# wagnva/semantic-nerf-for-satellite-data

Hardware: AMD Instinct MI355X
Metric: train rays/sec (4096 rays x 64 samples) (higher is better)
Workload: dtype f32(f16x2)

## Files before the change

### semantic-nerf-for-satellite-data_amd/csrc/api.hip

```cpp
#include <stdarg.h>
#include <stdio.h>
#include <stdlib.h>
#include <string.h>

#include <mutex>

#include "aux_kernels.h"
#include "bsp.h"
#include "composite.h"
#include "gemm.h"
#include "plan.h"

namespace snerf {

int forward_bsp(const Plan& p, const float* pk, const SnerfInputs* in, const SnerfOutputs* out, void* workspace, hipStream_t st);
int backward_bsp(const Plan& p, const float* pk, const SnerfInputs* in, const SnerfOutGrads* go, float* gp, float* d_t, float* d_t_s,
                 void* workspace, hipStream_t st);

static thread_local char g_err[512] = "";
void set_error(const char* fmt, ...) {
  va_list ap;
  va_start(ap, fmt);
  vsnprintf(g_err, sizeof(g_err), fmt, ap);
  va_end(ap);
// ... 269 lines not shown
namespace {
struct BufNote { const void* p; bool composed; };
constexpr int NOTE_MAX = 256;
BufNote g_notes[NOTE_MAX];
int g_n_notes = 0, g_note_next = 0;
std::mutex g_note_mu;
void note_plan(const void* buf, bool composed) {
  std::lock_guard<std::mutex> lk(g_note_mu);
  for (int i = 0; i < g_n_notes; ++i) if (g_notes[i].p == buf) { g_notes[i].composed = composed; return; }
  if (g_n_notes < NOTE_MAX) g_notes[g_n_notes++] = {buf, composed};
  else { g_notes[g_note_next] = {buf, composed}; g_note_next = (g_note_next + 1) % NOTE_MAX; }
}
int check_plan_note(const void* buf, bool composed, const char* who, const char* what) {
  std::lock_guard<std::mutex> lk(g_note_mu);
  for (int i = 0; i < g_n_notes; ++i)
    if (g_notes[i].p == buf && g_notes[i].composed != composed) {
      set_error("%s: the %s was written under SNERF_COMPOSE_FEATS=%d, this call is planned with %d (pack, forward and backward must agree)",
                who, what, g_notes[i].composed ? 1 : 0, composed ? 1 : 0);
      return SNERF_ERR_BAD_DESC;
    }
  return SNERF_OK;
}
}

static int check_inputs(const Plan& p, const SnerfInputs* in) {
  if (!in) { set_error("null inputs"); return SNERF_ERR_NULL; }
  if (!in->sun_d || in->sun_stride < 3) { set_error("sun_d (N,3) with stride >= 3 is required"); return SNERF_ERR_NULL; }
  if (!in->t) { set_error("t (N,tau) is required"); return SNERF_ERR_NULL; }
  if (p.x_ts >= 0 && !in->t_s) { set_error("t_s is required with use_separate_tj_for_semantic"); return SNERF_ERR_NULL; }
  if (in->xyz) {
    if (!in->z_vals) { set_error("explicit xyz needs explicit z_vals"); return SNERF_ERR_NULL; }
  } else {
    if (!in->rays) { set_error("rays or xyz is required"); return SNERF_ERR_NULL; }
    if (!in->z_vals && !in->z_steps) { set_error("z_steps is required when z_vals is not given"); return SNERF_ERR_NULL; }
  }
  return SNERF_OK;
}

}

using namespace snerf;

extern "C" {

int snerf_version(void) { return SNERF_ABI_VERSION; }
const char* snerf_last_error(void) { return g_err; }

size_t snerf_packed_floats(const SnerfDesc* desc) {
  Plan p;
  if (make_plan(desc, &p)) return 0;
  return p.packed_floats;
}

size_t snerf_grad_floats(const SnerfDesc* desc) {
  Plan p;
  if (make_plan(desc, &p)) return 0;
  return p.n_fp32;
}

size_t snerf_workspace_bytes(const SnerfDesc* desc) {
  Plan p;
  if (make_plan(desc, &p)) return 0;
  return p.ws_bytes;
}

int snerf_pack_params(const SnerfDesc* desc, const SnerfParams* params, float* packed, void* stream) {
  Plan p;
  RC(make_plan(desc, &p));
  if (!params || !packed) { set_error("null params/packed"); return SNERF_ERR_NULL; }
  TableBuilder tb;
  build_tables(p, params, tb);
  if (tb.missing) { set_error("snerf_pack_params: a parameter tensor required by this SnerfDesc is NULL"); return SNERF_ERR_NULL; }
  hipStream_t st = (hipStream_t)stream;
  RC(launch_zero_bytes(packed, p.n_fp32 * sizeof(float), st));
  for (int i = 0; i < tb.nt; ++i) RC(launch_copy_table(tb.tabs[i], packed, 0, st));
  char* planes = reinterpret_cast<char*>(packed + p.n_fp32);
  int* exps = reinterpret_cast<int*>(planes + p.wp_bytes);
  unsigned* maxbits = reinterpret_cast<unsigned*>(exps + bsp::WPACK_MAX);
  note_plan(packed, p.compose_feats);
  if (!p.compose_feats) return bsp::launch_wpack(p.wj, packed, planes, exps, maxbits, p.pl, st);
  {
    bsp::SgTable tb;
    bsp::compose_jobs(tb, packed + p.w_h1, packed + p.w_fs, packed + p.b_fs, packed + p.b_h1, packed + p.o_wc, packed + p.o_bc, p.W, p.FA, p.N1);
    RC(bsp::launch_sgemm(tb, 64, st));
  }
  bsp::WPackTable first, rest;
  first.n = rest.n = 0;
  for (int i = 0; i < p.wj.n; ++i) (i < p.wj_first ? first.j[first.n++] : rest.j[rest.n++]) = p.wj.j[i];
  RC(bsp::launch_wpack(first, packed, planes, exps, maxbits, p.pl, st));
  return bsp::launch_wpack(rest, packed, planes, exps, maxbits, p.pl, st);
}

int snerf_unpack_grads(const SnerfDesc* desc, const float* packed_grads, const SnerfParams* grads, int accumulate,
                       void* stream) {
  Plan p;
  RC(make_plan(desc, &p));
  if (!grads || !packed_grads) { set_error("null grads"); return SNERF_ERR_NULL; }
  TableBuilder tb;
  build_tables(p, grads, tb);
  if (tb.missing) { set_error("snerf_unpack_grads: a gradient tensor required by this SnerfDesc is NULL"); return SNERF_ERR_NULL; }
  hipStream_t st = (hipStream_t)stream;
  for (int i = 0; i < tb.nt; ++i) RC(launch_copy_table(tb.tabs[i], const_cast<float*>(packed_grads), accumulate ? 2 : 1, st));
  return SNERF_OK;
}

int snerf_forward(const SnerfDesc* desc, const float* packed_params, const SnerfInputs* in, const SnerfOutputs* out,
                  void* workspace, size_t workspace_bytes, void* stream) {
  Plan p;
  RC(make_plan(desc, &p));
  if (!packed_params || !out || !workspace) { set_error("snerf_forward: null argument"); return SNERF_ERR_NULL; }
  if (workspace_bytes < p.ws_bytes) { set_error("snerf_forward: workspace too small (%zu < %zu)", workspace_bytes, p.ws_bytes); return SNERF_ERR_WORKSPACE; }
  if (((uintptr_t)workspace & 255) || ((uintptr_t)packed_params & 255)) { set_error("workspace and packed params must be 256-byte aligned"); return SNERF_ERR_WORKSPACE; }
  RC(check_inputs(p, in));
  RC(check_plan_note(packed_params, p.compose_feats, "snerf_forward", "packed parameter buffer"));
  note_plan(workspace, p.compose_feats);
  return forward_bsp(p, packed_params, in, out, workspace, (hipStream_t)stream);
}

int snerf_backward(const SnerfDesc* desc, const float* packed_params, const SnerfInputs* in, const SnerfOutGrads* gout,
                   float* packed_grads, float* d_t, float* d_t_s, void* workspace, size_t workspace_bytes, void* stream) {
  Plan p;
  RC(make_plan(desc, &p));
  if (!p.train) { set_error("snerf_backward needs the SnerfDesc used for the SNERF_FLAG_TRAIN forward"); return SNERF_ERR_BAD_DESC; }
  if (!packed_params || !gout || !packed_grads || !workspace) { set_error("snerf_backward: null argument"); return SNERF_ERR_NULL; }
  if (workspace_bytes < p.ws_bytes) { set_error("snerf_backward: workspace too small (%zu < %zu)", workspace_bytes, p.ws_bytes); return SNERF_ERR_WORKSPACE; }
  if (((uintptr_t)workspace & 255) || ((uintptr_t)packed_params & 255) || ((uintptr_t)packed_grads & 255)) { set_error("workspace and packed buffers must be 256-byte aligned"); return SNERF_ERR_WORKSPACE; }
  RC(check_inputs(p, in));
  RC(check_plan_note(packed_params, p.compose_feats, "snerf_backward", "packed parameter buffer"));
  RC(check_plan_note(workspace, p.compose_feats, "snerf_backward", "workspace"));
  return backward_bsp(p, packed_params, in, gout, packed_grads, d_t, d_t_s, workspace, (hipStream_t)stream);
}

int snerf_sample_z(const float* rays, const float* z_steps, const float* u, float* z, int n_rays, int n_samples, void* stream) {
  if (!rays || !z_steps || !z || n_rays <= 0 || n_samples <= 0) { set_error("snerf_sample_z: bad argument"); return SNERF_ERR_NULL; }
  return launch_sample_z(rays, z_steps, u, z, n_rays, n_samples, (hipStream_t)stream);
}

int snerf_embedding_rows(const float* table, int n_embed, int tau, const long long* idx, int n, float* rows, void* stream) {
  if (!table || !idx || !rows || n_embed <= 0 || tau <= 0 || n <= 0) { set_error("snerf_embedding_rows: bad argument"); return SNERF_ERR_NULL; }
  return launch_embedding_rows(table, n_embed, tau, idx, n, rows, (hipStream_t)stream);
}

int snerf_embedding_backward(const long long* idx, const float* d_rows, int n, int tau, int n_embed, float* grad_table, void* stream) {
  if (!idx || !d_rows || !grad_table || n_embed <= 0 || tau <= 0 || n <= 0) { set_error("snerf_embedding_backward: bad argument"); return SNERF_ERR_NULL; }
  return launch_embedding_backward(idx, d_rows, n, tau, n_embed, grad_table, (hipStream_t)stream);
}

int snerf_profile_begin(void) { return profile_begin(); }
int snerf_profile_end(SnerfProfile* out) { return profile_end(out); }

}
```

### semantic-nerf-for-satellite-data_amd/csrc/bsp.h

```cpp
#pragma once
#include "common.h"
#include "gemm.h"

namespace snerf {
namespace bsp {

constexpr int RB = 128;
constexpr int CB = 128;
constexpr int E_MAX = 100;
constexpr int E_QUIET = 60;

typedef __amdgpu_buffer_rsrc_t srd_t;
typedef unsigned int u32x4 __attribute__((ext_vector_type(4)));
typedef unsigned int u32x2 __attribute__((ext_vector_type(2)));
typedef _Float16 f16x8 __attribute__((ext_vector_type(8)));
typedef _Float16 f16x4 __attribute__((ext_vector_type(4)));
constexpr unsigned OOB = 0xFFFFFFF0u;

__host__ __device__ inline int ncb_of(int ld) { return (ld + CB - 1) / CB; }
__host__ __device__ inline size_t plane_bytes(size_t rows, int ld, int pl = 2) { return rows * (size_t)ld * 2 * pl; }
__host__ __device__ inline size_t etab_ints(size_t rows, int ld) { return ((rows + RB - 1) / RB) * (size_t)ncb_of(ld); }
__host__ __device__ inline unsigned g16_off(int k, int pl = 2) { return (unsigned)(k >> 4) * 32u * (unsigned)pl + (unsigned)(k & 15) * 2u; }

__host__ __device__ inline int exp_of_maxbits(unsigned b) {
// ... 77 lines not shown
  float* colsum = nullptr; int ldcs = 0;
  int tiles_i = 0, tiles_j = 0;
  int tj_skip = -1;
  int tiles_jr = 0;
  int rev = 0;
  int dbg = 0;
  int* tile_ctr = nullptr;
  int pl = 2;
  const float* nd_w = nullptr; float* nd_out = nullptr; unsigned long long nd_stride = 0;
  int nd_omax = 0, nd_ldw = 0;
  int nd_rows[8] = {0, 0, 0, 0, 0, 0, 0, 0}, nd_row0[8] = {0, 0, 0, 0, 0, 0, 0, 0}, nd_woff[8] = {0, 0, 0, 0, 0, 0, 0, 0};
};
__host__ __device__ inline size_t sign_words(size_t rows, int ld) { return ((rows + 31) / 32) * (size_t)((ld + 63) / 64) * 64; }

struct DwArgs {
  const char* A = nullptr; const int* EA = nullptr; int lda = 0; int a_col0 = 0;
  const char* B = nullptr; const int* EB = nullptr; int ldb = 0; int b_col0 = 0;
  int I = 0, J = 0, P = 0;
  float* C = nullptr; int ldc = 0;
  int k_split = 0, n_split = 1; unsigned long long slab_stride = 0;
  int tiles_i = 0, tiles_j = 0;
  int pl = 2;
};

constexpr int TR_MAXL = 8;
constexpr int TR_SLOTS = TR_MAXL + 1;
struct TrunkArgs {
  const char* pe = nullptr; const int* Epe = nullptr;
  int P = 0, W = 0, L = 0; unsigned skip_mask = 0;
  int gamma_free_layer = 0;
  const char* Wp[TR_SLOTS] = {}; const int* EW[TR_SLOTS] = {}; unsigned w_bytes[TR_SLOTS] = {}; int K[TR_SLOTS] = {};
  const float* bias[TR_SLOTS] = {}; float w0[TR_SLOTS] = {};
  char* F = nullptr; int* EF = nullptr; int ldf = 0;
  char* H[TR_MAXL] = {}; int* EH[TR_MAXL] = {}; unsigned* Hsign[TR_MAXL] = {};
  const float* nd_w = nullptr; float* nd_out = nullptr; unsigned long long nd_stride = 0;
  int* tile_ctr = nullptr;
  int dbg = 0;
};
inline int trunk_gamma_free_layer(int L, unsigned skip_mask) {
  int g = 2;
  for (int l = 2; l < L; ++l)
    if ((skip_mask >> l) & 1u) g = l;
  return g < L - 1 ? g : L - 1;
}
inline bool trunk_dma_in_final_layer(int L, unsigned skip_mask, bool feats_fused) {
  return !feats_fused && trunk_gamma_free_layer(L, skip_mask) == L - 1;
}
int launch_trunk(const TrunkArgs& a, bool train, hipStream_t st);
void trunk_set_grid_override(int n);
void trunk_set_fusion(int on);
bool trunk_fusion_enabled();

int launch_kc(const KcArgs& a, hipStream_t st);
void kc_set_grid_override(int n);
int launch_kc_narrow(const KcArgs& a, hipStream_t st);
int launch_dw(const DwArgs& a, bool narrow_i, hipStream_t st);

int launch_to_planes(const float* src, int ld_src, int rows, int cols, char* dst, int* E, int ld, int col0, int pl, hipStream_t st);
int launch_from_planes(const char* src, const int* E, int ld, int col0, int rows, int cols, float* dst, int ld_dst, int pl, hipStream_t st);

struct WPackJob {
  unsigned long long src_off;
  int src_ld;
  int rows, K;
  int transposed;
  unsigned long long dst_off;
  int e_idx;
  int m_rows, m_cols;
};
constexpr int WPACK_MAX = 48;
struct WPackTable { WPackJob j[WPACK_MAX]; int n; };
constexpr int WPACK_CHUNK = 24;
struct WPackChunk { WPackJob j[WPACK_CHUNK]; int n; };
__host__ __device__ inline size_t wp16_bytes(int rows, int K, int pl = 2) { return (size_t)((rows + 31) / 32) * (size_t)(K / 16) * 1024 * pl; }
int launch_wpack(const WPackTable& tb, const float* master, char* planes, int* exps, unsigned* maxbits, int pl, hipStream_t st);

struct SgJob {
  const float* A = nullptr; long long sa_i = 0, sa_k = 0;
  const float* B = nullptr; long long sb_k = 0, sb_j = 0;
  const float* D = nullptr; int ldd = 0;
  const float* u = nullptr; const float* v = nullptr;
  float* C = nullptr; int ldc = 0;
  int M = 0, N = 0, K = 0, acc = 0;
  int blk0 = 0;
};
constexpr int SG_MAX = 6;
struct SgTable { SgJob j[SG_MAX]; int n = 0; };
int launch_sgemm(const SgTable& tb, int tile_m, hipStream_t st);
void compose_jobs(SgTable& tb, const float* w_h1, const float* w_f, const float* b_f, const float* b_h1, float* wc, float* bc, int W, int FA, int N1);
void uncompose_jobs(SgTable& tb, const float* G, const float* gc, const float* w_h1, const float* w_f, const float* b_f,
                    float* dw_h1, float* db_h1, float* dw_f, float* db_f, int W, int FA, int M);

}
struct EncodeArgs;
namespace bsp {
int launch_encode_bsp(const EncodeArgs& a, char* pe, int* Epe, char* fa, int* Efa, int fa_col0, int pl, hipStream_t st);
int launch_zero_cols(char* base, size_t pitch, size_t width_bytes, int rows, hipStream_t st);
int launch_colsum32_bsp(const float* in, int rows, float* partial, char* planes, int* E, int pl, hipStream_t st);

}
}
```

### semantic-nerf-for-satellite-data_amd/csrc/bsp_aux.hip

```cpp
#include "bsp.h"
#include "aux_kernels.h"

namespace snerf {
namespace bsp {

__device__ __forceinline__ float block_max_256(float m, float* sm) {
#pragma unroll
  for (int o = 32; o >= 1; o >>= 1) m = fmaxf(m, __shfl_xor(m, o, 64));
  __syncthreads();
  if ((threadIdx.x & 63) == 0) sm[threadIdx.x >> 6] = m;
  __syncthreads();
  return fmaxf(fmaxf(sm[0], sm[1]), fmaxf(sm[2], sm[3]));
}

__global__ __launch_bounds__(256) void to_planes_kernel(const float* __restrict__ src, int ld_src, int rows, int cols,
                                                        char* __restrict__ dst, int* __restrict__ E, int ld, int col0, int pl) {
  __shared__ float sm[4];
  const int rb = blockIdx.y, cb = blockIdx.x;
  const int t = threadIdx.x, c8 = cb * 128 + (t & 15) * 8;
  float v[8][8];
  float m = 0.f;
#pragma unroll
  for (int i = 0; i < 8; ++i) {
    const int r = rb * 128 + (t >> 4) + 16 * i;
// ... 26 lines not shown
    set_error("to_planes: bad argument (ld % 16, col0 % 128)");
    return SNERF_ERR_BAD_DESC;
  }
  hipLaunchKernelGGL(to_planes_kernel, dim3((cols + 127) / 128, (rows + 127) / 128), dim3(256), 0, st, src, ld_src, rows, cols,
                     dst, E, ld, col0, pl);
  SNERF_LAUNCH_CHECK();
  return SNERF_OK;
}

__global__ void from_planes_kernel(const char* __restrict__ src, const int* __restrict__ E, int ld, int col0, int rows, int cols,
                                   float* __restrict__ dst, int ld_dst, int pl) {
  const size_t g = (size_t)blockIdx.x * blockDim.x + threadIdx.x;
  if (g >= (size_t)rows * cols) return;
  const int r = (int)(g / cols), c = (int)(g - (size_t)r * cols);
  const char* p = src + (size_t)r * ld * 2 * pl + g16_off(col0 + c, pl);
  const float hi = (float)*reinterpret_cast<const _Float16*>(p), lo = pl == 2 ? (float)*reinterpret_cast<const _Float16*>(p + 32) : 0.f;
  const int e = E[(size_t)(r >> 7) * ncb_of(ld) + ((col0 + c) >> 7)];
  dst[(size_t)r * ld_dst + c] = __builtin_amdgcn_ldexpf(hi + lo, -e);
}

int launch_from_planes(const char* src, const int* E, int ld, int col0, int rows, int cols, float* dst, int ld_dst, int pl, hipStream_t st) {
  const size_t n = (size_t)rows * cols;
  hipLaunchKernelGGL(from_planes_kernel, dim3((unsigned)((n + 255) / 256)), dim3(256), 0, st, src, E, ld, col0, rows, cols, dst, ld_dst, pl);
  SNERF_LAUNCH_CHECK();
  return SNERF_OK;
}

__global__ __launch_bounds__(256) void wmax_kernel(WPackChunk tb, const float* __restrict__ master, unsigned* __restrict__ maxbits) {
  const WPackJob j = tb.j[blockIdx.y];
  if (j.transposed == 1) return;
  float m = 0.f;
  const int wave = threadIdx.x >> 6, lane = threadIdx.x & 63;
  for (int r = blockIdx.x * 4 + wave; r < j.m_rows; r += gridDim.x * 4) {
    const float* row = master + j.src_off + (size_t)r * j.src_ld;
    for (int c = lane; c < j.m_cols; c += 64) m = fmaxf(m, fabsf(row[c]));
  }
#pragma unroll
  for (int o = 32; o >= 1; o >>= 1) m = fmaxf(m, __shfl_xor(m, o, 64));
  if ((threadIdx.x & 63) == 0 && m > 0.f) atomicMax(maxbits + j.e_idx, __float_as_uint(m));
}

__global__ __launch_bounds__(256) void wpack_kernel(WPackChunk tb, const float* __restrict__ master, char* __restrict__ planes,
                                                    int* __restrict__ exps, const unsigned* __restrict__ maxbits, int pl) {
  const WPackJob j = tb.j[blockIdx.y];
  const int rb32 = (j.rows + 31) >> 5, nks = j.K >> 4;
  const int e = exp_of_maxbits(maxbits[j.e_idx]);
  if (blockIdx.x == 0 && threadIdx.x == 0) exps[j.e_idx] = e;
  const float sc = pow2f(e);
  for (int unit = blockIdx.x; unit < rb32 * nks; unit += gridDim.x) {
    const int ks = unit / rb32, ub = unit - ks * rb32;
    const int r = threadIdx.x >> 3, kp = (threadIdx.x & 7) * 2;
    const int ra = ub * 32 + wf16_row(r), ka = ks * 16 + kp;
    float x[2];
#pragma unroll
    for (int q = 0; q < 2; ++q) {
      const int k = ka + q;
      const bool ok = j.transposed ? (k < j.m_rows && ra < j.m_cols) : (ra < j.m_rows && k < j.m_cols);
      x[q] = ok ? master[j.src_off + (j.transposed ? (size_t)k * j.src_ld + ra : (size_t)ra * j.src_ld + k)] : 0.f;
    }
    const _Float16 h0 = (_Float16)(x[0] * sc), h1 = (_Float16)(x[1] * sc);
    const _Float16 l0 = (_Float16)(x[0] * sc - (float)h0), l1 = (_Float16)(x[1] * sc - (float)h1);
    typedef _Float16 f16x2 __attribute__((ext_vector_type(2)));
    char* u = planes + j.dst_off + (size_t)unit * 1024 * pl + (32 * (kp >> 3) + r) * 16 + (kp & 7) * 2;
    *reinterpret_cast<f16x2*>(u) = f16x2{h0, h1};
    if (pl == 2) *reinterpret_cast<f16x2*>(u + 1024) = f16x2{l0, l1};
  }
}

int launch_wpack(const WPackTable& tb, const float* master, char* planes, int* exps, unsigned* maxbits, int pl, hipStream_t st) {
  if (tb.n <= 0) return SNERF_OK;
  { int rc = launch_zero_bytes(maxbits, WPACK_MAX * sizeof(unsigned), st); if (rc) return rc; }
  for (int pass = 0; pass < 2; ++pass)
    for (int first = 0; first < tb.n; first += WPACK_CHUNK) {
      WPackChunk c;
      c.n = tb.n - first < WPACK_CHUNK ? tb.n - first : WPACK_CHUNK;
      for (int i = 0; i < c.n; ++i) c.j[i] = tb.j[first + i];
      if (pass == 0) hipLaunchKernelGGL(wmax_kernel, dim3(32, c.n), dim3(256), 0, st, c, master, maxbits);
      else hipLaunchKernelGGL(wpack_kernel, dim3(128, c.n), dim3(256), 0, st, c, master, planes, exps, maxbits, pl);
      SNERF_LAUNCH_CHECK();
    }
  return SNERF_OK;
}

template <int TM>
__global__ __launch_bounds__(256) void sgemm_jobs_kernel(const SgTable tb) {
  constexpr int BM = 16 * TM, BN = 64, BK = 16;
  __shared__ float As[BK][BM + 1];
  __shared__ float Bs[BK][BN + 4];
  int q = 0;
  while (q + 1 < tb.n && (int)blockIdx.x >= tb.j[q + 1].blk0) ++q;
  const SgJob jb = tb.j[q];
  const int tiles_n = (jb.N + BN - 1) / BN;
  const int tile = (int)blockIdx.x - jb.blk0;
  const int i0 = (tile / tiles_n) * BM, j0 = (tile % tiles_n) * BN;
  const int t = threadIdx.x, ty = t >> 4, tx = t & 15;
  float acc[TM][4];
#pragma unroll
  for (int r = 0; r < TM; ++r)
#pragma unroll
    for (int c = 0; c < 4; ++c) acc[r][c] = 0.f;
  const bool a_k_fast = jb.sa_k == 1, b_j_fast = jb.sb_j == 1;
  for (int k0 = 0; k0 < jb.K; k0 += BK) {
#pragma unroll
    for (int s = 0; s < (BM * BK) / 256; ++s) {
      const int idx = t + 256 * s;
      const int i = a_k_fast ? idx / BK : idx % BM, k = a_k_fast ? idx % BK : idx / BM;
      As[k][i] = (i0 + i < jb.M && k0 + k < jb.K) ? jb.A[(long long)(i0 + i) * jb.sa_i + (long long)(k0 + k) * jb.sa_k] : 0.f;
    }
#pragma unroll
    for (int s = 0; s < (BN * BK) / 256; ++s) {
      const int idx = t + 256 * s;
      const int j = b_j_fast ? idx % BN : idx / BK, k = b_j_fast ? idx / BN : idx % BK;
      Bs[k][j] = (j0 + j < jb.N && k0 + k < jb.K) ? jb.B[(long long)(k0 + k) * jb.sb_k + (long long)(j0 + j) * jb.sb_j] : 0.f;
    }
    __syncthreads();
#pragma unroll
    for (int k = 0; k < BK; ++k) {
      float a[TM], b[4];
#pragma unroll
      for (int r = 0; r < TM; ++r) a[r] = As[k][ty * TM + r];
#pragma unroll
      for (int c = 0; c < 4; ++c) b[c] = Bs[k][tx * 4 + c];
#pragma unroll
      for (int r = 0; r < TM; ++r)
#pragma unroll
        for (int c = 0; c < 4; ++c) acc[r][c] = fmaf(a[r], b[c], acc[r][c]);
    }
    __syncthreads();
  }
#pragma unroll
  for (int r = 0; r < TM; ++r) {
    const int i = i0 + ty * TM + r;
    if (i >= jb.M) continue;
#pragma unroll
    for (int c = 0; c < 4; ++c) {
      const int j = j0 + tx * 4 + c;
      if (j >= jb.N) continue;
      float x = acc[r][c];
      if (jb.u) x = fmaf(jb.u[i], jb.v[j], x);
      if (jb.D) x += jb.D[(size_t)i * jb.ldd + j];
      float* o = jb.C + (size_t)i * jb.ldc + j;
      *o = jb.acc ? *o + x : x;
    }
  }
}

void compose_jobs(SgTable& tb, const float* w_h1, const float* w_f, const float* b_f, const float* b_h1, float* wc, float* bc, int W, int FA, int N1) {
  const int X = FA - W;
  tb.n = 0;
  auto job = [&]() -> SgJob& { tb.j[tb.n] = SgJob(); return tb.j[tb.n++]; };
  { SgJob& j = job(); j.A = w_h1; j.sa_i = FA; j.sa_k = 1; j.B = w_f; j.sb_k = W; j.sb_j = 1; j.C = wc; j.ldc = FA; j.M = N1; j.N = W; j.K = W; }
  { SgJob& j = job(); j.D = w_h1 + W; j.ldd = FA; j.C = wc + W; j.ldc = FA; j.M = N1; j.N = X; }
  { SgJob& j = job(); j.D = w_f + (size_t)W * W; j.ldd = W; j.C = wc + (size_t)N1 * FA; j.ldc = FA; j.M = 32; j.N = W; }
  { SgJob& j = job(); j.C = wc + (size_t)N1 * FA + W; j.ldc = FA; j.M = 32; j.N = X; }
  { SgJob& j = job(); j.A = w_h1; j.sa_i = FA; j.sa_k = 1; j.B = b_f; j.sb_k = 1; j.sb_j = 0; j.D = b_h1; j.ldd = 1; j.C = bc; j.ldc = 1; j.M = N1; j.N = 1; j.K = W; }
}
void uncompose_jobs(SgTable& tb, const float* G, const float* gc, const float* w_h1, const float* w_f, const float* b_f,
                    float* dw_h1, float* db_h1, float* dw_f, float* db_f, int W, int FA, int M) {
  tb.n = 0;
  auto job = [&]() -> SgJob& { tb.j[tb.n] = SgJob(); return tb.j[tb.n++]; };
  { SgJob& j = job(); j.A = G; j.sa_i = FA; j.sa_k = 1; j.B = w_f; j.sb_k = 1; j.sb_j = W; j.u = gc; j.v = b_f; j.C = dw_h1; j.ldc = FA; j.M = M; j.N = W; j.K = W; j.acc = 1; }
  { SgJob& j = job(); j.A = w_h1; j.sa_i = 1; j.sa_k = FA; j.B = G; j.sb_k = FA; j.sb_j = 1; j.C = dw_f; j.ldc = W; j.M = W; j.N = W; j.K = M; j.acc = 1; }
  { SgJob& j = job(); j.A = w_h1; j.sa_i = 1; j.sa_k = FA; j.B = gc; j.sb_k = 1; j.sb_j = 0; j.C = db_f; j.ldc = 1; j.M = W; j.N = 1; j.K = M; j.acc = 1; }
  { SgJob& j = job(); j.D = gc; j.ldd = 1; j.C = db_h1; j.ldc = 1; j.M = M; j.N = 1; j.acc = 1; }
}

int launch_sgemm(const SgTable& tb0, int tile_m, hipStream_t st) {
  if (tb0.n <= 0) return SNERF_OK;
  if (tb0.n > SG_MAX || (tile_m != 64 && tile_m != 32)) { set_error("sgemm: bad job table"); return SNERF_ERR_BAD_DESC; }
  SgTable tb = tb0;
  int blocks = 0;
  for (int q = 0; q < tb.n; ++q) {
    SgJob& j = tb.j[q];
    if (!j.C || j.M <= 0 || j.N <= 0 || j.K < 0 || j.ldc < 1 || (j.K > 0 && (!j.A || !j.B)) || (j.u && !j.v) || (j.D && j.ldd < 1)) {
      set_error("sgemm: bad job %d", q);
      return SNERF_ERR_BAD_DESC;
    }
    j.blk0 = blocks;
    blocks += ((j.M + tile_m - 1) / tile_m) * ((j.N + 63) / 64);
  }
  if (tile_m == 64) hipLaunchKernelGGL(sgemm_jobs_kernel<4>, dim3(blocks), dim3(256), 0, st, tb);
  else hipLaunchKernelGGL(sgemm_jobs_kernel<2>, dim3(blocks), dim3(256), 0, st, tb);
  SNERF_LAUNCH_CHECK();
  return SNERF_OK;
}

__global__ void zero_cols_kernel(char* base, size_t pitch, int width16, int rows) {
  const int i = blockIdx.x * blockDim.x + threadIdx.x;
  if (i >= rows * width16) return;
  const int r = i / width16, c = i - r * width16;
  *reinterpret_cast<u32x4*>(base + (size_t)r * pitch + 16 * (size_t)c) = u32x4{0u, 0u, 0u, 0u};
}
int launch_zero_cols(char* base, size_t pitch, size_t width_bytes, int rows, hipStream_t st) {
  const int w16 = (int)(width_bytes / 16);
  if (w16 <= 0 || rows <= 0) return SNERF_OK;
  hipLaunchKernelGGL(zero_cols_kernel, dim3((unsigned)(((size_t)rows * w16 + 255) / 256)), dim3(256), 0, st, base, pitch, w16, rows);
  SNERF_LAUNCH_CHECK();
  return SNERF_OK;
}

__device__ __forceinline__ void point_xyz(const EncodeArgs& a, long long point, float (&x)[3]) {
  const int n = (int)((unsigned)point / (unsigned)a.S);
#pragma unroll
  for (int c = 0; c < 3; ++c) {
    if (a.xyz != nullptr) {
      x[c] = a.xyz[point * 3 + c];
    } else {
#pragma clang fp contract(off)
      const float o = a.rays[n * 8 + c];
      const float d = a.dir_is_sun ? a.sun_d[(size_t)n * a.sun_stride + c] : a.rays[n * 8 + 3 + c];
      const float dz = d * a.z[point];
      x[c] = o + dz;
    }
  }
}
__device__ __forceinline__ float extras_value(const EncodeArgs& a, int n, int c) {
  if (c >= a.x_sun && c < a.x_sun + 3) return a.sun_d[(size_t)n * a.sun_stride + (c - a.x_sun)];
  if (a.t != nullptr && c >= a.x_t && c < a.x_t + a.tau) return a.t[(size_t)n * a.tau + (c - a.x_t)];
  if (a.t_s != nullptr && a.x_ts >= 0 && c >= a.x_ts && c < a.x_ts + a.tau) return a.t_s[(size_t)n * a.tau + (c - a.x_ts)];
  return 0.f;
}

struct EncodeBsp {
  EncodeArgs a;
  char* pe; int* Epe;
  char* fa; int* Efa; int fa_col0;
  int pl;
};

__global__ __launch_bounds__(256) void encode_bsp_kernel(EncodeBsp g) {
  __shared__ float sm[4];
  const EncodeArgs& a = g.a;
  const int rb = blockIdx.x, t = threadIdx.x;
  if (rb == 0) for (int i = t; i < a.zero_n; i += 256) a.zero[i] = 0u;
  const long long P = (long long)a.N * a.S;
  const long long p0 = (long long)rb * 128;
  const int npts = (int)min((long long)128, P - p0);
  float mx = 0.f, me = 0.f;
  if (a.F == 0)
    for (int i = t; i < npts; i += 256) {
      float x[3];
      point_xyz(a, p0 + i, x);
      mx = fmaxf(mx, fmaxf(fabsf(x[0]), fmaxf(fabsf(x[1]), fabsf(x[2]))));
    }
  if (g.fa != nullptr) {
    const int n0 = (int)((unsigned)p0 / (unsigned)a.S), n1 = (int)((unsigned)(p0 + npts - 1) / (unsigned)a.S);
    for (int i = t; i < (n1 - n0 + 1) * 16; i += 256) me = fmaxf(me, fabsf(extras_value(a, n0 + (i >> 4), i & 15)));
  }
  const int e_pe = a.F > 0 ? 13 : exp_of_maxbits(__float_as_uint(block_max_256(mx, sm)));
  const int e_x = g.fa != nullptr ? exp_of_maxbits(__float_as_uint(block_max_256(me, sm))) : 0;
  if (t == 0) {
    g.Epe[rb] = e_pe;
    if (g.fa != nullptr) g.Efa[(size_t)rb * ncb_of(a.FA) + (g.fa_col0 >> 7)] = e_x;
  }
  const float s_pe = pow2f(e_pe), s_x = pow2f(e_x);
  const int gpe = a.Ep >> 4, ngrp = gpe + (g.fa != nullptr ? 1 : 0);
  for (int item = t; item < npts * ngrp; item += 256) {
    const int pl = item / ngrp, grp = item - pl * ngrp;
    const long long point = p0 + pl;
    float v[16];
    char* d;
    float sc;
    if (grp < gpe) {
      float x[3];
      point_xyz(a, point, x);
// ... 118 lines not shown
```

### semantic-nerf-for-satellite-data_amd/csrc/bsp_pass.hip

```cpp
#include "aux_kernels.h"
#include "bsp.h"
#include "composite.h"
#include "plan.h"

namespace snerf {

namespace {
struct Ws {
  char* base;
  char* c(size_t off) const { return base + off; }
  float* f(size_t off) const { return reinterpret_cast<float*>(base + off); }
  int* i(size_t off) const { return reinterpret_cast<int*>(base + off); }
  unsigned* u(size_t off) const { return reinterpret_cast<unsigned*>(base + off); }
  void a(bsp::KcArgs& g, const PlaneT& t, int k, int col0 = 0) const { g.A = c(t.o); g.EA = i(t.e); g.lda = t.ld; g.a_col0 = col0; g.Ka = k; }
  void a2(bsp::KcArgs& g, const PlaneT& t) const { g.A2 = c(t.o); g.EA2 = i(t.e); g.lda2 = t.ld; }
  void out(bsp::KcArgs& g, const PlaneT& t, int col0 = 0) const { g.C = c(t.o); g.EC = i(t.e); g.ldc = t.ld; g.c_col0 = col0; g.Csign = t.s ? u(t.s) : nullptr; }
  void h(bsp::KcArgs& g, const PlaneT& t, int col0 = 0) const { g.H = c(t.o); g.EH = i(t.e); g.ldh = t.ld; g.h_col0 = col0; g.Hsign = t.s ? u(t.s) : nullptr; }
  void dz(bsp::DwArgs& g, const PlaneT& t) const { g.A = c(t.o); g.EA = i(t.e); g.lda = t.ld; g.a_col0 = 0; }
  void x(bsp::DwArgs& g, const PlaneT& t, int col0) const { g.B = c(t.o); g.EB = i(t.e); g.ldb = t.ld; g.b_col0 = col0; }
};
struct WOp { const char* W; const int* EW; int rb32; unsigned bytes; int K; };
WOp wop(const Plan& p, const float* pk, int job) {
  const char* planes = reinterpret_cast<const char*>(pk + p.n_fp32);
  const bsp::WPackJob& w = p.wj.j[job];
// ... 315 lines not shown
    const int r0 = p.sc ? p.sun_col : 0;
    const int nt = (P + 127) / 128, X = p.FA - W;
    RC(dw_gemm(r.w_h1, dz1, p.h1w, false, p.fa, 0, p.FA));
    RC(red_add_elem2d(rq.elem, r.w_h1.slab + W, r.w_h1.sp.ns, r.w_h1.stride, p.h1w, X, p.FA, gp + p.w_h1 + (size_t)r0 * p.FA + W, p.FA));
    RC(red_add_elem2d(rq.elem, r.w_h1.slab, r.w_h1.sp.ns, r.w_h1.stride, p.h1w, W, p.FA, r.w_h1.slab, p.FA));
    RC(red_store_last(rq.elem));
    RC(red_add_col(rq.col, r.cs_fin, nt, (size_t)r.ld_cs1, p.h1w, r.cs_fin));
    RC(red_store_last(rq.col));
    uncompose = true;
    RC(transient_grads());
    if (sig_live) {
      RC(narrow_grad(dsig, r.nar_sig, p.pdsig, gp + p.b_fs + W));
      RC(dw_gemm(r.w_fs, p.pdsig, NARROW, true, hl, 0, W));
      RC(dw_reduce(r.w_fs, (size_t)NARROW * W, gp + p.w_fs + (size_t)W * W));
    }
    { const PlaneT sw = dz_cur; dz_cur = dz_nxt; dz_nxt = sw; }
    bsp::KcArgs g;
    ws.a(g, dz1, p.h1w);
    if (sig_live) ws.a2(g, p.pdsig);
    weights(g, p, pk, p.wj_th1, 0, r0); g.I = P; g.J = W; g.K = sig_live ? p.h1w + NARROW : p.h1w;
    ws.out(g, dz_cur);
    dact(g, hl, 0, (p.L == 1) ? 30.f : 1.f);
    colsum(g, r.cs_hl, W);
    RC(launch_kc(g));
    RC(bias_from_colsum(r.cs_hl, W, gp + p.b_tr[p.L - 1]));
  }
  const PlaneT dfa = p.dzb.view(p.FA);
  if (!p.compose_feats) {
    const int r0 = p.sc ? p.sun_col : 0;
    RC(dw_gemm(r.w_h1, dz1, p.h1w, false, p.fa, 0, p.FA));
    RC(dw_reduce(r.w_h1, (size_t)p.h1w * p.FA, gp + p.w_h1 + (size_t)r0 * p.FA));
    bsp::KcArgs g;
    ws.a(g, dz1, p.h1w); weights(g, p, pk, p.wj_th1, 0, r0);
    g.I = P; g.J = W; g.K = p.h1w; ws.out(g, dfa);
    colsum(g, r.cs_fa, p.FA);
    RC(launch_kc(g));
    RC(red_add_col(rq.col, r.cs_fa, (P + 127) / 128, (size_t)cs_ld(p.FA), W, gp + p.b_fs));
    RC(transient_grads());
  }
  if (!p.compose_feats) {
    if (sig_live) RC(narrow_grad(dsig, r.nar_sig, p.pdsig, gp + p.b_fs + W));
    RC(dw_gemm(r.w_fs, dfa, W, false, hl, 0, W));
    if (sig_live) RC(dw_gemm(r.w_fs, p.pdsig, NARROW, true, hl, 0, W, (size_t)W * W));
    RC(dw_reduce(r.w_fs, (size_t)(sig_live ? W + NARROW : W) * W, gp + p.w_fs));
    bsp::KcArgs g;
    ws.a(g, dfa, W);
    if (sig_live) ws.a2(g, p.pdsig);
    weights(g, p, pk, p.wj_tfs); g.I = P; g.J = W; g.K = sig_live ? W + NARROW : W;
    ws.out(g, dz_cur);
    dact(g, hl, 0, (p.L == 1) ? 30.f : 1.f);
    colsum(g, r.cs_hl, W);
    RC(launch_kc(g));
    RC(bias_from_colsum(r.cs_hl, W, gp + p.b_tr[p.L - 1]));
  }
  for (int i = p.L - 1; i >= 0; --i) {
    const BwdRegions::Layer& t = r.tr[i];
    if (i > 0 && ((p.skip_mask >> i) & 1u)) {
      RC(dw_gemm(t.w_gamma, dz_cur, W, false, p.pe, 0, p.Ep));
      RC(dw_gemm(t.w, dz_cur, W, false, p.h[i - 1], 0, W));
      RC(red_add_elem2d(rq.elem, t.w_gamma.slab, t.w_gamma.sp.ns, t.w_gamma.stride, W, p.Ep, p.Ep, gp + p.w_tr[i], p.k_tr[i]));
      RC(red_add_elem2d(rq.elem, t.w.slab, t.w.sp.ns, t.w.stride, W, W, W, gp + p.w_tr[i] + p.Ep, p.k_tr[i]));
    } else {
      if (i == 0) RC(dw_gemm(t.w, dz_cur, W, false, p.pe, 0, p.Ep));
      else RC(dw_gemm(t.w, dz_cur, W, false, p.h[i - 1], 0, W));
      RC(dw_reduce(t.w, (size_t)W * p.k_tr[i], gp + p.w_tr[i]));
    }
    if (i == 0) break;
    bsp::KcArgs g;
    ws.a(g, dz_cur, W); weights(g, p, pk, p.wj_tt[i]);
    g.I = P; g.J = W; g.K = W; ws.out(g, dz_nxt);
    dact(g, p.h[i - 1], 0, (i - 1 == 0) ? 30.f : 1.f);
    colsum(g, t.cs, W);
    RC(launch_kc(g));
    RC(bias_from_colsum(t.cs, W, gp + p.b_tr[i - 1]));
    const PlaneT sw = dz_cur; dz_cur = dz_nxt; dz_nxt = sw;
  }
  RC(launch_reductions(rq.elem, rq.col, st));
  if (!uncompose) return SNERF_OK;
  {
    const size_t r0 = p.sc ? (size_t)p.sun_col : 0;
    bsp::SgTable tb;
    bsp::uncompose_jobs(tb, r.w_h1.slab, r.cs_fin, pk + p.w_h1 + r0 * p.FA, pk + p.w_fs, pk + p.b_fs,
                        gp + p.w_h1 + r0 * p.FA, gp + p.b_h1 + r0, gp + p.w_fs, gp + p.b_fs, W, p.FA, p.h1w);
    return bsp::launch_sgemm(tb, 32, st);
  }
}

}
```

Before: 170,500.

## Rewrite FP32 job-table SGEMM with double-buffered register prefetch and per-job tile size

```diff
diff --git a/semantic-nerf-for-satellite-data_amd/csrc/api.hip b/semantic-nerf-for-satellite-data_amd/csrc/api.hip
--- a/semantic-nerf-for-satellite-data_amd/csrc/api.hip
+++ b/semantic-nerf-for-satellite-data_amd/csrc/api.hip
@@ -375,7 +375,7 @@
   {
     bsp::SgTable tb;
     bsp::compose_jobs(tb, packed + p.w_h1, packed + p.w_fs, packed + p.b_fs, packed + p.b_h1, packed + p.o_wc, packed + p.o_bc, p.W, p.FA, p.N1);
-    RC(bsp::launch_sgemm(tb, 64, st));
+    RC(bsp::launch_sgemm(tb, st));
   }
   bsp::WPackTable first, rest;
   first.n = rest.n = 0;
diff --git a/semantic-nerf-for-satellite-data_amd/csrc/bsp.h b/semantic-nerf-for-satellite-data_amd/csrc/bsp.h
--- a/semantic-nerf-for-satellite-data_amd/csrc/bsp.h
+++ b/semantic-nerf-for-satellite-data_amd/csrc/bsp.h
@@ -183,11 +183,11 @@
   const float* u = nullptr; const float* v = nullptr;
   float* C = nullptr; int ldc = 0;
   int M = 0, N = 0, K = 0, acc = 0;
-  int blk0 = 0;
+  int blk0 = 0, tm = 0;
 };
 constexpr int SG_MAX = 6;
 struct SgTable { SgJob j[SG_MAX]; int n = 0; };
-int launch_sgemm(const SgTable& tb, int tile_m, hipStream_t st);
+int launch_sgemm(const SgTable& tb, hipStream_t st);
 void compose_jobs(SgTable& tb, const float* w_h1, const float* w_f, const float* b_f, const float* b_h1, float* wc, float* bc, int W, int FA, int N1);
 void uncompose_jobs(SgTable& tb, const float* G, const float* gc, const float* w_h1, const float* w_f, const float* b_f,
                     float* dw_h1, float* db_h1, float* dw_f, float* db_f, int W, int FA, int M);
diff --git a/semantic-nerf-for-satellite-data_amd/csrc/bsp_aux.hip b/semantic-nerf-for-satellite-data_amd/csrc/bsp_aux.hip
--- a/semantic-nerf-for-satellite-data_amd/csrc/bsp_aux.hip
+++ b/semantic-nerf-for-satellite-data_amd/csrc/bsp_aux.hip
@@ -132,16 +132,53 @@
   return SNERF_OK;
 }
 
+constexpr int SG_T = 128, SG_BN = 64, SG_BK = 32;
+
+template <int X>
+__device__ __forceinline__ void sg_load(const float* __restrict__ P, long long sx, long long sk, bool kfast, bool vec, int x0, int k0,
+                                        int XN, int K, int t, float4 (&r)[X / 16]) {
+  const int dx = kfast ? 0 : 1, dk = 1 - dx;
+  const long long se = kfast ? sk : sx;
+#pragma unroll
+  for (int s = 0; s < X / 16; ++s) {
+    const int idx = t + SG_T * s;
+    const int x = kfast ? idx % X : (idx % (X / 4)) * 4, k = kfast ? (idx / X) * 4 : idx / (X / 4);
+    const long long off = (long long)(x0 + x) * sx + (long long)(k0 + k) * sk;
+    if (vec) {
+      r[s] = *reinterpret_cast<const float4*>(P + off);
+    } else {
+      float e[4];
+#pragma unroll
+      for (int q = 0; q < 4; ++q) {
+        const bool ok = (x0 + x + q * dx < XN) & (k0 + k + q * dk < K);
+        const float v = P[ok ? off + q * se : 0];
+        e[q] = ok ? v : 0.f;
+      }
+      r[s] = make_float4(e[0], e[1], e[2], e[3]);
+    }
+  }
+}
+template <int X>
+__device__ __forceinline__ void sg_store(float* __restrict__ S, bool kfast, int t, const float4 (&r)[X / 16]) {
+#pragma unroll
+  for (int s = 0; s < X / 16; ++s) {
+    const int idx = t + SG_T * s;
+    if (kfast) {
+      const int x = idx % X, k = (idx / X) * 4;
+      S[(k + 0) * X + x] = r[s].x; S[(k + 1) * X + x] = r[s].y; S[(k + 2) * X + x] = r[s].z; S[(k + 3) * X + x] = r[s].w;
+    } else {
+      *reinterpret_cast<float4*>(S + (idx / (X / 4)) * X + (idx % (X / 4)) * 4) = r[s];
+    }
+  }
+}
+__device__ __forceinline__ bool sg_vec_ok(const float* P, long long s_unit, long long s_other) {
+  return s_unit == 1 && (s_other & 3) == 0 && (reinterpret_cast<size_t>(P) & 15) == 0;
+}
+
 template <int TM>
-__global__ __launch_bounds__(256) void sgemm_jobs_kernel(const SgTable tb) {
-  constexpr int BM = 16 * TM, BN = 64, BK = 16;
-  __shared__ float As[BK][BM + 1];
-  __shared__ float Bs[BK][BN + 4];
-  int q = 0;
-  while (q + 1 < tb.n && (int)blockIdx.x >= tb.j[q + 1].blk0) ++q;
-  const SgJob jb = tb.j[q];
+__device__ __forceinline__ void sg_tile(const SgJob& jb, int tile, float* __restrict__ As, float* __restrict__ Bs) {
+  constexpr int BM = 8 * TM, BN = SG_BN, BK = SG_BK;
   const int tiles_n = (jb.N + BN - 1) / BN;
-  const int tile = (int)blockIdx.x - jb.blk0;
   const int i0 = (tile / tiles_n) * BM, j0 = (tile % tiles_n) * BN;
   const int t = threadIdx.x, ty = t >> 4, tx = t & 15;
   float acc[TM][4];
@@ -149,34 +186,39 @@
   for (int r = 0; r < TM; ++r)
 #pragma unroll
     for (int c = 0; c < 4; ++c) acc[r][c] = 0.f;
-  const bool a_k_fast = jb.sa_k == 1, b_j_fast = jb.sb_j == 1;
-  for (int k0 = 0; k0 < jb.K; k0 += BK) {
-#pragma unroll
-    for (int s = 0; s < (BM * BK) / 256; ++s) {
-      const int idx = t + 256 * s;
-      const int i = a_k_fast ? idx / BK : idx % BM, k = a_k_fast ? idx % BK : idx / BM;
-      As[k][i] = (i0 + i < jb.M && k0 + k < jb.K) ? jb.A[(long long)(i0 + i) * jb.sa_i + (long long)(k0 + k) * jb.sa_k] : 0.f;
-    }
-#pragma unroll
-    for (int s = 0; s < (BN * BK) / 256; ++s) {
-      const int idx = t + 256 * s;
-      const int j = b_j_fast ? idx % BN : idx / BK, k = b_j_fast ? idx / BN : idx % BK;
-      Bs[k][j] = (j0 + j < jb.N && k0 + k < jb.K) ? jb.B[(long long)(k0 + k) * jb.sb_k + (long long)(j0 + j) * jb.sb_j] : 0.f;
-    }
+  const bool a_kfast = jb.sa_k == 1, b_kfast = jb.sb_j != 1;
+  const bool a_vec = i0 + BM <= jb.M && (a_kfast ? sg_vec_ok(jb.A, jb.sa_k, jb.sa_i) : sg_vec_ok(jb.A, jb.sa_i, jb.sa_k));
+  const bool b_vec = j0 + BN <= jb.N && (b_kfast ? sg_vec_ok(jb.B, jb.sb_k, jb.sb_j) : sg_vec_ok(jb.B, jb.sb_j, jb.sb_k));
+  const int nsteps = (jb.K + BK - 1) / BK;
+  float4 ra[BM / 16], rb[BN / 16];
+  if (nsteps > 0) {
+    sg_load<BM>(jb.A, jb.sa_i, jb.sa_k, a_kfast, false, i0, 0, jb.M, jb.K, t, ra);
+    sg_load<BN>(jb.B, jb.sb_j, jb.sb_k, b_kfast, false, j0, 0, jb.N, jb.K, t, rb);
+  }
+  for (int s = 0; s < nsteps; ++s) {
+    sg_store<BM>(As + (s & 1) * (BK * BM), a_kfast, t, ra);
+    sg_store<BN>(Bs + (s & 1) * (BK * BN), b_kfast, t, rb);
     __syncthreads();
-#pragma unroll
+    if (s + 1 < nsteps) {
+      const int k0 = (s + 1) * BK;
+      const bool full = k0 + BK <= jb.K;
+      sg_load<BM>(jb.A, jb.sa_i, jb.sa_k, a_kfast, a_vec && full, i0, k0, jb.M, jb.K, t, ra);
+      sg_load<BN>(jb.B, jb.sb_j, jb.sb_k, b_kfast, b_vec && full, j0, k0, jb.N, jb.K, t, rb);
+    }
+    const float* as = As + (s & 1) * (BK * BM) + ty * TM;
+    const float* bs = Bs + (s & 1) * (BK * BN) + tx * 4;
+#pragma unroll 8
     for (int k = 0; k < BK; ++k) {
-      float a[TM], b[4];
-#pragma unroll
-      for (int r = 0; r < TM; ++r) a[r] = As[k][ty * TM + r];
-#pragma unroll
-      for (int c = 0; c < 4; ++c) b[c] = Bs[k][tx * 4 + c];
+      float a[TM];
+      if constexpr (TM == 4) { const float4 v = *reinterpret_cast<const float4*>(as + k * BM); a[0] = v.x; a[1] = v.y; a[2] = v.z; a[3] = v.w; }
+      else { const float2 v = *reinterpret_cast<const float2*>(as + k * BM); a[0] = v.x; a[1] = v.y; }
+      const float4 bv = *reinterpret_cast<const float4*>(bs + k * BN);
+      const float b[4] = {bv.x, bv.y, bv.z, bv.w};
 #pragma unroll
       for (int r = 0; r < TM; ++r)
 #pragma unroll
         for (int c = 0; c < 4; ++c) acc[r][c] = fmaf(a[r], b[c], acc[r][c]);
     }
-    __syncthreads();
   }
 #pragma unroll
   for (int r = 0; r < TM; ++r) {
@@ -193,6 +235,17 @@
       *o = jb.acc ? *o + x : x;
     }
   }
+}
+
+__global__ __launch_bounds__(SG_T) void sgemm_jobs_kernel(const SgTable tb) {
+  __shared__ __attribute__((aligned(16))) float As[2 * SG_BK * 32];
+  __shared__ __attribute__((aligned(16))) float Bs[2 * SG_BK * SG_BN];
+  int q = 0;
+  while (q + 1 < tb.n && (int)blockIdx.x >= tb.j[q + 1].blk0) ++q;
+  const SgJob jb = tb.j[q];
+  const int tile = (int)blockIdx.x - jb.blk0;
+  if (jb.tm == 2) sg_tile<2>(jb, tile, As, Bs);
+  else sg_tile<4>(jb, tile, As, Bs);
 }
 
 void compose_jobs(SgTable& tb, const float* w_h1, const float* w_f, const float* b_f, const float* b_h1, float* wc, float* bc, int W, int FA, int N1) {
@@ -215,9 +268,9 @@
   { SgJob& j = job(); j.D = gc; j.ldd = 1; j.C = db_h1; j.ldc = 1; j.M = M; j.N = 1; j.acc = 1; }
 }
 
-int launch_sgemm(const SgTable& tb0, int tile_m, hipStream_t st) {
+int launch_sgemm(const SgTable& tb0, hipStream_t st) {
   if (tb0.n <= 0) return SNERF_OK;
-  if (tb0.n > SG_MAX || (tile_m != 64 && tile_m != 32)) { set_error("sgemm: bad job table"); return SNERF_ERR_BAD_DESC; }
+  if (tb0.n > SG_MAX) { set_error("sgemm: bad job table"); return SNERF_ERR_BAD_DESC; }
   SgTable tb = tb0;
   int blocks = 0;
   for (int q = 0; q < tb.n; ++q) {
@@ -226,11 +279,11 @@
       set_error("sgemm: bad job %d", q);
       return SNERF_ERR_BAD_DESC;
     }
+    j.tm = j.K > 512 ? 2 : 4;
     j.blk0 = blocks;
-    blocks += ((j.M + tile_m - 1) / tile_m) * ((j.N + 63) / 64);
-  }
-  if (tile_m == 64) hipLaunchKernelGGL(sgemm_jobs_kernel<4>, dim3(blocks), dim3(256), 0, st, tb);
-  else hipLaunchKernelGGL(sgemm_jobs_kernel<2>, dim3(blocks), dim3(256), 0, st, tb);
+    blocks += ((j.M + 8 * j.tm - 1) / (8 * j.tm)) * ((j.N + SG_BN - 1) / SG_BN);
+  }
+  hipLaunchKernelGGL(sgemm_jobs_kernel, dim3(blocks), dim3(SG_T), 0, st, tb);
   SNERF_LAUNCH_CHECK();
   return SNERF_OK;
 }
diff --git a/semantic-nerf-for-satellite-data_amd/csrc/bsp_pass.hip b/semantic-nerf-for-satellite-data_amd/csrc/bsp_pass.hip
--- a/semantic-nerf-for-satellite-data_amd/csrc/bsp_pass.hip
+++ b/semantic-nerf-for-satellite-data_amd/csrc/bsp_pass.hip
@@ -421,8 +421,8 @@
     bsp::SgTable tb;
     bsp::uncompose_jobs(tb, r.w_h1.slab, r.cs_fin, pk + p.w_h1 + r0 * p.FA, pk + p.w_fs, pk + p.b_fs,
                         gp + p.w_h1 + r0 * p.FA, gp + p.b_h1 + r0, gp + p.w_fs, gp + p.b_fs, W, p.FA, p.h1w);
-    return bsp::launch_sgemm(tb, 32, st);
-  }
-}
-
-}
+    return bsp::launch_sgemm(tb, st);
+  }
+}
+
+}
```

Result: no change. 170,800, median of 6 (+0.1%).
